# hellojialee/OffsetGuided

Measured on AMD Instinct MI355X. Metric: images/sec end-to-end (backbone+decode) @640x640 bs8; decoder-only ms/img, higher is better.
Workload: dtype f16

## Files before the change

include/og_decoder.h:

```cpp
#ifndef OG_DECODER_H
#define OG_DECODER_H

#include <stddef.h>
#include <stdint.h>

#ifdef __cplusplus
extern "C" {
#endif

#define OG_ABI_VERSION 4

#define OG_OK 0
#define OG_EINVAL (-1)
#define OG_ENOSPC (-2)
#define OG_EHIP (-3)
#define OG_EUNSUPPORTED (-4)

int og_abi_version(void);
const char *og_last_error(void);

int og_device_count(void);

int og_upsample_bicubic4_f32(const float *src, long planes, int h, int w, float *dst, void *stream);

// ... 82 lines not shown
int og_upsample2_add_bf16(void *up, const void *low, long n, int H, int W, int channels, void *stream);

int og_nchw_f32_to_nhwc_bf16(const float *src, void *dst, long N, int C, int H, int W, void *stream);
int og_nhwc_bf16_to_nchw_f32(const void *src, int src_channels, int first_channel, int channels, const float *bias,
                             float *dst, long N, int H, int W, void *stream);

int og_center_pad_normalize_u8(const unsigned char *img, int h, int w, int target_h, int target_w, const float *mean3,
                               const float *std3, const float *fill3, float *out, int *ltrb, void *stream);

int og_resize_cubic_u8(const unsigned char *src, int h, int w, unsigned char *dst, int new_h, int new_w, void *stream);

int og_shrink_mask_miss_u8(const unsigned char *mask, int N, int h, int w, int stride, unsigned char *out, void *stream);

int og_rescale_pad_normalize_u8(const unsigned char *img, int h, int w, int new_h, int new_w, int target_h, int target_w,
                                int corner_pad, const float *mean3, const float *std3, const float *fill3, float *out,
                                int *ltrb, void *stream);

int og_rescale_pad_normalize_batch_u8(const unsigned char *raw, const long *offsets, const int *hw4, int n, int target_h,
                                      int target_w, int corner_pad, const float *mean3, const float *std3, const float *fill3,
                                      float *out, int *ltrb, void *stream);

int og_stem7x7_bf16(const float *images, const void *w_packed, const float *bias, void *out, int N, int H, int W, int relu,
                    void *stream);

int og_conv3x3_bf16(const void *x, const void *w, const float *bias, const void *skip, void *out, int N, int H, int W,
                    int Cin, int Cout, int relu, void *workspace, size_t workspace_bytes, void *stream);
size_t og_conv3x3_workspace_bytes(long pixels, int Cin, int Cout);
size_t og_conv3x3_workspace_bytes_nhw(int N, int H, int W, int Cin, int Cout);
int og_conv2d_bf16(const void *x, const void *w, const float *bias, const void *skip, void *out, int N, int Hin, int Win,
                   int Cin, int Cout, int ksize, int stride, int relu, void *workspace, size_t workspace_bytes,
                   void *stream);
size_t og_conv2d_workspace_bytes(int N, int Hin, int Win, int Cin, int Cout, int ksize, int stride);
int og_conv2d_proj_bf16(const void *x, const void *w_cat, const float *bias, const void *x2, void *out, int N, int Hin,
                        int Win, int Cin, int Cout, int ksize, int stride, int H2, int W2, int Cin2, int stride2, int relu,
                        void *workspace, size_t workspace_bytes, void *stream);
size_t og_conv2d_proj_workspace_bytes(int N, int Hin, int Win, int Cin, int Cout, int ksize, int stride, int Cin2);
int og_conv_band_supported(int N, int Hin, int Win, int Cin, int Cout, int stride, int H2, int W2, int Cin2, int stride2);
int og_conv_band_pack_w16(const void *w, const void *w2, int Cin, int Cout, int Cin2, void *packed, void *stream);
int og_conv_band_bf16(const void *x, const void *w_packed, const float *bias, const void *skip, const void *x2, void *out, int N,
                      int Hin, int Win, int Cin, int Cout, int stride, int relu, int H2, int W2, int Cin2, int stride2, void *stream);
int og_conv_band_f16(const void *x, const void *w_packed, const float *bias, const void *skip, const void *x2, void *out, int N,
                     int Hin, int Win, int Cin, int Cout, int stride, int relu, int H2, int W2, int Cin2, int stride2, void *stream);
void og_conv_next_weights_hint(const void *w_next, size_t bytes);
int og_conv3x3_tiled_supported(int N, int H, int W, int Cin, int Cout);
int og_conv3x3_pack_w16(const void *w, int Cin, int Cout, int order, void *packed, void *stream);
size_t og_conv3x3_tiled_workspace_bytes(int N, int H, int W, int Cin, int Cout);
int og_conv3x3_tiled_bf16(const void *x, const void *w_packed, const float *bias, const void *skip, void *out, int N, int H,
                          int W, int Cin, int Cout, int relu, void *workspace, size_t workspace_bytes, void *stream);
int og_conv3x3_tiled_up2_bf16(const void *x, const void *w_packed, const float *bias, const void *skip, void *up, int N, int H,
                              int W, int Cin, int Cout, int relu, void *workspace, size_t workspace_bytes, void *stream);
int og_conv3x3s2_tiled_supported(int N, int Hin, int Win, int Cin, int Cout);
int og_conv3x3s2_tiled_bf16(const void *x, const void *w_packed, const float *bias, const void *skip, void *out, int N, int Hin,
                            int Win, int Cin, int Cout, int relu, void *stream);
int og_conv1x1_tiled_bf16(const void *x1, int C1, int H1, int W1, int stride1, const void *x2, int C2, int H2, int W2, int stride2,
                          const void *w_packed, const float *bias, const void *skip, void *out, int N, int H, int W, int Cout,
                          int relu, void *stream);
int og_conv1x1_heads_bf16(const void *x, int C, const void *w_packed, const float *bias, int N, int H, int W, int Cout, int n_heads,
                          const int *head_channels, float *const *outs, void *stream);
int og_bias_act_f16(void *x, const float *bias, const void *skip, long pixels, int channels, int relu, void *stream);
int og_upsample2_add_f16(void *up, const void *low, long n, int H, int W, int channels, void *stream);
int og_nchw_f32_to_nhwc_f16(const float *src, void *dst, long N, int C, int H, int W, void *stream);
int og_nhwc_f16_to_nchw_f32(const void *src, int src_channels, int first_channel, int channels, const float *bias,
                            float *dst, long N, int H, int W, void *stream);
int og_stem7x7_f16(const float *images, const void *w_packed, const float *bias, void *out, int N, int H, int W, int relu,
                   void *stream);
int og_conv3x3_f16(const void *x, const void *w, const float *bias, const void *skip, void *out, int N, int H, int W,
                   int Cin, int Cout, int relu, void *workspace, size_t workspace_bytes, void *stream);
int og_conv3x3_tiled_f16(const void *x, const void *w_packed, const float *bias, const void *skip, void *out, int N, int H,
                         int W, int Cin, int Cout, int relu, void *workspace, size_t workspace_bytes, void *stream);
int og_conv3x3_tiled_up2_f16(const void *x, const void *w_packed, const float *bias, const void *skip, void *up, int N, int H,
                         int W, int Cin, int Cout, int relu, void *workspace, size_t workspace_bytes, void *stream);
int og_conv3x3s2_tiled_f16(const void *x, const void *w_packed, const float *bias, const void *skip, void *out, int N, int Hin,
                           int Win, int Cin, int Cout, int relu, void *stream);
int og_conv1x1_tiled_f16(const void *x1, int C1, int H1, int W1, int stride1, const void *x2, int C2, int H2, int W2, int stride2,
                         const void *w_packed, const float *bias, const void *skip, void *out, int N, int H, int W, int Cout,
                         int relu, void *stream);
int og_conv1x1_heads_f16(const void *x, int C, const void *w_packed, const float *bias, int N, int H, int W, int Cout, int n_heads,
                         const int *head_channels, float *const *outs, void *stream);
int og_conv2d_f16(const void *x, const void *w, const float *bias, const void *skip, void *out, int N, int Hin, int Win,
                  int Cin, int Cout, int ksize, int stride, int relu, void *workspace, size_t workspace_bytes, void *stream);
int og_conv2d_proj_f16(const void *x, const void *w_cat, const float *bias, const void *x2, void *out, int N, int Hin,
                       int Win, int Cin, int Cout, int ksize, int stride, int H2, int W2, int Cin2, int stride2, int relu,
                       void *workspace, size_t workspace_bytes, void *stream);

int og_focal_l2_loss_f32(const float *pred, const float *gt, const unsigned char *mask_miss, int N, int C, long hw,
                         float tau, float gamma, float *sum, float *grad, void *stream);
int og_offset_l1_loss_f32(const float *pred, const float *gt, const float *gt_ps, const unsigned char *mask_miss, int N,
                          int C, long hw, float margin, int sqrt_re, float *sum_count, float *grad, void *stream);
int og_l2_loss_f32(const float *pred, const float *gt, const unsigned char *mask_miss, int N, int C, long hw, float *sum,
                   float *grad, void *stream);
int og_masked_l1_loss_f32(const float *pred, const float *gt, const unsigned char *mask_miss, int N, int C, long hw,
                          float margin, int sqrt_re, float *sum_count, float *grad, void *stream);
int og_vector_l1_loss_f32(const float *pred, const float *gt, const unsigned char *mask_miss, int N, int C, long hw,
                          float margin, int sqrt_re, float *sum_count, float *grad, void *stream);
int og_laplace_loss_f32(const float *pred, const float *gt, const float *logb, const unsigned char *mask_miss, int N, int C,
                        long hw, float margin, int sqrt_re, float *sum_count, float *grad, float *grad_logb, void *stream);

int og_encode_heatmaps_f32(const float *joints, const int32_t *n_persons, int N, int P, int n_kp, int in_w, int in_h,
                           int stride, int sigma, float clip_thre, float *hm, float *bg, void *stream);
int og_encode_jitter_f32(const float *joints, const int32_t *n_persons, int N, int P, int n_kp, int in_w, int in_h,
                         int stride, int fill_size, float *jit, void *stream);
int og_encode_offsets_f32(const float *joints, const int32_t *n_persons, int N, int P, int n_kp, const int32_t *jf,
                          const int32_t *jt, int L, int in_w, int in_h, int stride, int fill_size, float min_jscale,
                          const float *sigmas, float *off, float *scale, float *pscale, void *stream);

int og_draw_poses_u8(void *images, const float *poses, const int *n_persons, const int *skeleton,
// ... 93 lines not shown
```

offsetguided_amd/_lib.py:

```python
import ctypes as C
import os

import torch

_HERE = os.path.dirname(os.path.abspath(__file__))
LIB_PATH = os.path.join(_HERE, "libog_decoder.so")
if os.environ.get("OG_DECODER_LIB"):
    LIB_PATH = os.environ["OG_DECODER_LIB"]

OG_OK, OG_EINVAL, OG_ENOSPC, OG_EHIP, OG_EUNSUPPORTED = 0, -1, -2, -3, -4
ABI_VERSION = 4

_vp, _i, _l, _f, _d, _sz = C.c_void_p, C.c_int, C.c_long, C.c_float, C.c_double, C.c_size_t


class LimbsDesc(C.Structure):
    _fields_ = [("size", C.c_uint32), ("hmps", _vp), ("hm_lowres", _i), ("kp_perm", _vp), ("offs", _vp), ("off_lowres", _i), ("vector_nd", _i),
                ("limb_perm", _vp), ("reserve_mask", _vp), ("score_ksize", _i), ("scales", _vp), ("scales_mode", _i), ("jitter", _vp),
                ("jitter_mode", _i), ("N", _i), ("C", _i), ("H", _i), ("W", _i), ("jf", _vp), ("jt", _vp), ("L", _i), ("k", _i),
                ("thre_hmp", _f), ("min_len", _f), ("resize_factor", _f), ("topk_scores", _vp), ("topk_inds", _vp), ("limbs", _vp)]

    def __init__(self, **fields):
        super().__init__(size=C.sizeof(LimbsDesc), **{k: v.data_ptr() if isinstance(v, torch.Tensor) else v for k, v in fields.items()})

# ... 5 lines not shown

    def __init__(self, **fields):
        super().__init__(size=C.sizeof(CocoMaskDesc), **{k: v.data_ptr() if isinstance(v, torch.Tensor) else v for k, v in fields.items()})


SIGNATURES = {
    "og_abi_version": (_i, []),
    "og_last_error": (C.c_char_p, []),
    "og_device_count": (_i, []),
    "og_upsample_bicubic4_f32": (_i, [_vp, _l, _i, _i, _vp, _vp]),
    "og_upsample_bilinear4_f32": (_i, [_vp, _l, _i, _i, _vp, _vp]),
    "og_upsample_bicubic4_flip_f32": (_i, [_vp, _vp, _i, _i, _i, _i, _vp, _vp]),
    "og_hmp_nms_f32": (_i, [_vp, _l, _i, _i, _vp, _vp]),
    "og_hmp_nms_k_f32": (_i, [_vp, _l, _i, _i, _i, _vp, _vp]),
    "og_topk_channel_f32": (_i, [_vp, _l, _i, _i, _i, _vp, _vp, _vp, _sz, _vp]),
    "og_nms_topk_f32": (_i, [_vp, _l, _i, _i, _i, _vp, _vp, _vp, _sz, _vp]),
    "og_scored_offset_f32": (_i, [_vp, _vp, _i, _i, _i, _i, _i, _vp, _i, _vp, _vp]),
    "og_upsample_nms_topk_f32": (_i, [_vp, _l, _i, _i, _i, _vp, _vp, _vp, _sz, _vp]),
    "og_topk_workspace_bytes": (_sz, [_l, _i, _i, _i]),
    "og_collect_limbs_f32": (_i, [_vp, _vp, C.POINTER(LimbsDesc), _vp]),
    "og_generate_limbs_f32": (_i, [C.POINTER(LimbsDesc), _vp, _sz, _vp]),
    "og_generate_limbs_workspace_bytes": (_sz, [_i, _i, _i, _i, _i]),
    "og_greedy_group_f32": (_i, [_vp, _i, _i, _i, _vp, _vp, _i, _d, _f, _i, _i, _i, _vp, _vp, _vp, _vp, _sz, _vp]),
    "og_group_workspace_bytes": (_sz, [_i, _i, _i, _i, _i]),
    "og_flip_merge_f32": (_i, [_vp, _vp, _i, _i, _i, _i, _i, _vp, _vp, _vp, _vp, _vp, _vp]),
    "og_flip_cat_f32": (_i, [_vp, _vp, _i, _i, _i, _i, _i, _vp, _vp, _vp, _vp, _vp, _vp]),
    "og_flip_merge_heads_f32": (_i, [_vp, _vp, _i, _i, _i, _i, _vp, _vp, _vp, _vp]),
    "og_scale_accumulate_f32": (_i, [_vp, _vp, _i, _i, _i, _i, _i, _i, _vp, _vp, _vp, _vp, _i, _i, _i, _f, _vp, _vp, _vp]),
    "og_scale_accumulate_heads_f32": (_i, [_vp, _vp, _vp, _vp, _i, _i, _i, _i, _i, _i, _vp, _vp, _vp, _vp, _i, _i, _i, _f, _vp, _vp, _vp, _vp,
                                           _vp]),
    "og_bias_act_bf16": (_i, [_vp, _vp, _vp, _l, _i, _i, _vp]),
    "og_upsample2_add_bf16": (_i, [_vp, _vp, _l, _i, _i, _i, _vp]),
    "og_nchw_f32_to_nhwc_bf16": (_i, [_vp, _vp, _l, _i, _i, _i, _vp]),
    "og_nhwc_bf16_to_nchw_f32": (_i, [_vp, _i, _i, _i, _vp, _vp, _l, _i, _i, _vp]),
    "og_center_pad_normalize_u8": (_i, [_vp, _i, _i, _i, _i, _vp, _vp, _vp, _vp, _vp, _vp]),
    "og_resize_cubic_u8": (_i, [_vp, _i, _i, _vp, _i, _i, _vp]),
    "og_shrink_mask_miss_u8": (_i, [_vp, _i, _i, _i, _i, _vp, _vp]),
    "og_rescale_pad_normalize_u8": (_i, [_vp, _i, _i, _i, _i, _i, _i, _i, _vp, _vp, _vp, _vp, _vp, _vp]),
    "og_rescale_pad_normalize_batch_u8": (_i, [_vp, _vp, _vp, _i, _i, _i, _i, _vp, _vp, _vp, _vp, _vp, _vp]),
    "og_stem7x7_bf16": (_i, [_vp, _vp, _vp, _vp, _i, _i, _i, _i, _vp]),
    "og_conv3x3_bf16": (_i, [_vp, _vp, _vp, _vp, _vp, _i, _i, _i, _i, _i, _i, _vp, _sz, _vp]),
    "og_conv3x3_workspace_bytes": (_sz, [_l, _i, _i]),
    "og_conv3x3_workspace_bytes_nhw": (_sz, [_i, _i, _i, _i, _i]),
    "og_conv2d_bf16": (_i, [_vp, _vp, _vp, _vp, _vp, _i, _i, _i, _i, _i, _i, _i, _i, _vp, _sz, _vp]),
    "og_conv2d_workspace_bytes": (_sz, [_i, _i, _i, _i, _i, _i, _i]),
    "og_conv2d_proj_bf16": (_i, [_vp, _vp, _vp, _vp, _vp, _i, _i, _i, _i, _i, _i, _i, _i, _i, _i, _i, _i, _vp, _sz, _vp]),
    "og_conv2d_proj_workspace_bytes": (_sz, [_i, _i, _i, _i, _i, _i, _i, _i]),
    "og_conv_band_supported": (_i, [_i, _i, _i, _i, _i, _i, _i, _i, _i, _i]),
    "og_conv_band_pack_w16": (_i, [_vp, _vp, _i, _i, _i, _vp, _vp]),
    "og_conv_band_bf16": (_i, [_vp, _vp, _vp, _vp, _vp, _vp, _i, _i, _i, _i, _i, _i, _i, _i, _i, _i, _i, _vp]),
    "og_conv3x3_tiled_supported": (_i, [_i, _i, _i, _i, _i]),
    "og_conv3x3_pack_w16": (_i, [_vp, _i, _i, _i, _vp, _vp]),
    "og_conv3x3s2_tiled_supported": (_i, [_i, _i, _i, _i, _i]),
    "og_conv1x1_tiled_bf16": (_i, [_vp, _i, _i, _i, _i, _vp, _i, _i, _i, _i, _vp, _vp, _vp, _vp, _i, _i, _i, _i, _i, _vp]),
    "og_conv1x1_heads_bf16": (_i, [_vp, _i, _vp, _vp, _i, _i, _i, _i, _i, _vp, _vp, _vp]),
    "og_conv3x3s2_tiled_bf16": (_i, [_vp, _vp, _vp, _vp, _vp, _i, _i, _i, _i, _i, _i, _vp]),
    "og_conv3x3_tiled_workspace_bytes": (_sz, [_i, _i, _i, _i, _i]),
    "og_conv_next_weights_hint": (None, [_vp, _sz]),
    "og_conv3x3_tiled_bf16": (_i, [_vp, _vp, _vp, _vp, _vp, _i, _i, _i, _i, _i, _i, _vp, _sz, _vp]),
    "og_conv3x3_tiled_up2_bf16": (_i, [_vp, _vp, _vp, _vp, _vp, _i, _i, _i, _i, _i, _i, _vp, _sz, _vp]),
    "og_encode_heatmaps_f32": (_i, [_vp, _vp, _i, _i, _i, _i, _i, _i, _i, _f, _vp, _vp, _vp]),
    "og_encode_jitter_f32": (_i, [_vp, _vp, _i, _i, _i, _i, _i, _i, _i, _vp, _vp]),
    "og_encode_offsets_f32": (_i, [_vp, _vp, _i, _i, _i, _vp, _vp, _i, _i, _i, _i, _i, _f, _vp, _vp, _vp, _vp, _vp]),
    "og_focal_l2_loss_f32": (_i, [_vp, _vp, _vp, _i, _i, _l, _f, _f, _vp, _vp, _vp]),
    "og_offset_l1_loss_f32": (_i, [_vp, _vp, _vp, _vp, _i, _i, _l, _f, _i, _vp, _vp, _vp]),
    "og_l2_loss_f32": (_i, [_vp, _vp, _vp, _i, _i, _l, _vp, _vp, _vp]),
    "og_masked_l1_loss_f32": (_i, [_vp, _vp, _vp, _i, _i, _l, _f, _i, _vp, _vp, _vp]),
    "og_vector_l1_loss_f32": (_i, [_vp, _vp, _vp, _i, _i, _l, _f, _i, _vp, _vp, _vp]),
    "og_laplace_loss_f32": (_i, [_vp, _vp, _vp, _vp, _i, _i, _l, _f, _i, _vp, _vp, _vp, _vp]),
    "og_draw_poses_u8": (_i, [_vp, _vp, _vp, _vp, _vp, _i, _i, _i, _i, _i, _i, _i, _f, _f, _f, _vp]),
    "og_draw_heatmap_u8": (_i, [_vp, _vp, _vp, _i, _i, _i, _i, _i, _i, _f, _f, _f, _i, _vp]),
    "og_draw_segments_u8": (_i, [_vp, _vp, _vp, _i, _i, _i, _i, C.c_uint, C.c_uint, _f, _f, _f, _f, _vp]),
    "og_limbs_to_segments_f32": (_i, [_vp, _i, _i, _i, _i, _f, _vp, _vp, _vp]),
    "og_offsets_segments_capacity": (_l, [_i, _i, _i]),
    "og_offsets_to_segments_f32": (_i, [_vp, _vp, _i, _i, _i, _i, _i, _i, _i, _i, _f, _vp, _vp, _vp]),
    "og_warp_affine_batch_u8": (_i, [_vp, _vp, _vp, _i, _vp, _i, _vp, _vp, _vp, _vp, _vp, _vp]),
    "og_warp_affine_mask_u8": (_i, [_vp, _vp, _vp, _i, _vp, _i, _i, _vp, _vp]),
    "og_affine_joints_f32": (_i, [_vp, _vp, _i, _i, _i, _vp, _vp, _vp, _f, _f, _vp, _vp, _i, _vp, _vp]),
    "og_warp_affine_photo_batch_u8": (_i, [_vp, _vp, _vp, _i, _vp, _i, _vp, _vp, _vp, _vp, _vp, _vp, _vp]),
    "og_jpeg_roundtrip_batch_u8": (_i, [_vp, _i, _i, _vp, _i, _i, _vp, _vp, _vp, _vp, _vp]),
    "og_affine_joints_jitter_f32": (_i, [_vp, _vp, _i, _i, _i, _vp, _vp, _vp, _f, _f, _vp, _vp, _i, _vp, _vp, _vp, _vp, _vp, _vp]),
    "og_oks_matrix_f64": (_i, [_vp, _vp, _vp, _vp, _vp, _vp, _vp, _vp, _i, _i, _i, C.c_int64, _vp, _vp]),
    "og_oks_match_workspace_bytes": (_sz, [_i, _i, _i]),
    "og_oks_match_i32": (_i, [_vp, _vp, _vp, _vp, _vp, _vp, _vp, _vp, _vp, _i, _vp, _i, _i, _i, _i, C.c_int64, _vp, _vp, _vp, _vp, _sz, _vp]),
    "og_coco_mask_workspace_bytes": (_sz, [C.POINTER(CocoMaskDesc)]),
    "og_coco_masks_u8": (_i, [C.POINTER(CocoMaskDesc), _vp, _sz, _vp]),
    "og_optim_chunk_elems": (_i, []),
    "og_optim_workspace_bytes": (_sz, [_i]),
    "og_grad_sumsq_f32": (_i, [_vp, _vp, _i, _i, _vp, _sz, _vp]),
    "og_step_scale_f32": (_i, [_i, _vp, _f, _f, _vp, _sz, _vp]),
    "og_step_scale_amp_f32": (_i, [_i, _vp, _f, _f, _vp, _i, _f, _i, _f, _f, _vp, _sz, _vp]),
    "og_adam_step_f32": (_i, [_vp, _vp, _i, _i, _i, _vp, _f, _f, _f, _f, _f, _f, _f, _f, _f, _i, _vp]),
    "og_sgd_step_f32": (_i, [_vp, _vp, _i, _i, _i, _vp, _f, _f, _f, _i, _vp]),
}

for _name in [n for n in SIGNATURES if n.endswith('_bf16')]:
    SIGNATURES[_name[:-5] + '_f16'] = SIGNATURES[_name]
SIGNATURES['og_nhwc_f16_to_nchw_f32'] = SIGNATURES['og_nhwc_bf16_to_nchw_f32']

_lib = None


def lp(lib, stem, dtype):
    return getattr(lib, stem + ('_f16' if dtype == torch.float16 else '_bf16'))


# ... 188 lines not shown
```

offsetguided_amd/csrc/conv3x3.hip:

```cpp
#include <stdio.h>

#include <type_traits>

#include "lp_dtype.h"
#include "og_common.h"

namespace {

typedef lp8 bf16x8;
typedef float f32x4 __attribute__((ext_vector_type(4)));
typedef unsigned short u16x4 __attribute__((ext_vector_type(4)));
typedef unsigned short u16x8 __attribute__((ext_vector_type(8)));

constexpr int kZeroPageBytes = 256;

struct ConvArgs {
    const unsigned short *x;
    const unsigned short *w;
    const float *bias;
    const unsigned short *skip;
    unsigned short *out;
    unsigned short *up;
    float *partial;
    int *counters;
// ... 635 lines not shown
    return OG_OK;
}
}

OG_API int OG_LP_NAME(og_conv3x3_tiled)(const void *x, const void *w_packed, const float *bias, const void *skip, void *out, int N,
                                        int H, int W, int Cin, int Cout, int relu, void *workspace, size_t workspace_bytes,
                                        void *stream)
{
    return conv3x3_tiled_impl(OG_LP_STR("og_conv3x3_tiled"), x, w_packed, bias, skip, out, nullptr, N, H, W, Cin, Cout, relu, workspace,
                              workspace_bytes, stream);
}

OG_API int OG_LP_NAME(og_conv3x3_tiled_up2)(const void *x, const void *w_packed, const float *bias, const void *skip, void *up, int N,
                                            int H, int W, int Cin, int Cout, int relu, void *workspace, size_t workspace_bytes,
                                            void *stream)
{
    const char *name = OG_LP_STR("og_conv3x3_tiled_up2");
    OG_REQUIRE(up, OG_EINVAL, "%s: null pointer", name);
    OG_REQUIRE((long)N * H * W * 4 * Cout < (1l << 30), OG_EUNSUPPORTED, "%s: tensor too large (>= 2 GiB)", name);
    return conv3x3_tiled_impl(name, x, w_packed, bias, skip, nullptr, up, N, H, W, Cin, Cout, relu, workspace, workspace_bytes, stream);
}

OG_API int OG_LP_NAME(og_conv3x3s2_tiled)(const void *x, const void *w_packed, const float *bias, const void *skip, void *out,
                                          int N, int Hin, int Win, int Cin, int Cout, int relu, void *stream)
{
    const char *name = OG_LP_STR("og_conv3x3s2_tiled");
    OG_REQUIRE(x && w_packed && bias && out, OG_EINVAL, "%s: null pointer", name);
    ConvArgs h = {};
    const int rc = tiled_fill(name, h, x, w_packed, bias, skip, out, N, Hin, Win, 2, Cin, Cout, relu);
    if (rc != OG_OK) return rc;
    const int kind = og_conv3x3s2_tiled_supported(N, Hin, Win, Cin, Cout);
    OG_REQUIRE(kind != 0, OG_EUNSUPPORTED,
               "%s: needs Cout %% 128 == 0, Cin %% 64 == 0 and an output of 8k x 16k pixels or 2k x 40 (got %dx%d -> %dx%d, %d -> %d)", name,
               Hin, Win, h.H, h.W, Cin, Cout);
    h.warm = og_take_warm_hint();
#define S2_LAUNCH(TW_, TH_, WM_)                                                                                      \
    do {                                                                                                              \
        static OgAttrOnce attr_;                                                                                      \
        if (attr_.need())                                                                                             \
            (void)hipFuncSetAttribute((const void *)conv3x3s2_tiled_kernel<TW_, TH_, WM_>,                            \
                                      hipFuncAttributeMaxDynamicSharedMemorySize, kS2LdsBytes);                       \
        const long blocks_ = (long)N * (h.H / TH_) * (h.W / TW_) * h.n_tiles;                                         \
        hipLaunchKernelGGL((conv3x3s2_tiled_kernel<TW_, TH_, WM_>), dim3((unsigned)blocks_), dim3(256), kS2LdsBytes,  \
                           (hipStream_t)stream, h);                                                                   \
    } while (0)
    if (kind == 2) S2_LAUNCH(40, 2, 1);
    else S2_LAUNCH(16, 8, 2);
#undef S2_LAUNCH
    OG_LAUNCH_CHECK(name);
    return OG_OK;
}

static int pw_fill(const char *name, PwArgs &a, const void *x1, int C1, int H1, int W1, int s1, const void *x2, int C2, int H2, int W2,
                   int s2, const void *w_packed, const float *bias, int N, int H, int W, int Cout, int bn)
{
    OG_REQUIRE(x1 && w_packed, OG_EINVAL, "%s: null pointer", name);
    OG_REQUIRE(N > 0 && H > 0 && W > 0 && (s1 == 1 || s1 == 2) && (!x2 || s2 == 1 || s2 == 2), OG_EINVAL, "%s: bad shape", name);
    OG_REQUIRE(C1 > 0 && C1 % 64 == 0 && (!x2 || (C2 > 0 && C2 % 64 == 0)) && Cout % bn == 0, OG_EUNSUPPORTED,
               "%s: input channels must be multiples of 64 and Cout of %d (got %d + %d -> %d)", name, bn, C1, x2 ? C2 : 0, Cout);
    OG_REQUIRE((H - 1) * s1 < H1 && (W - 1) * s1 < W1, OG_EINVAL, "%s: the strided output reaches outside the input", name);
    OG_REQUIRE(!x2 || (C2 == C1 && H2 == H1 && W2 == W1 && s2 == s1), OG_EUNSUPPORTED,
               "%s: a second input must have the shape and stride of the first", name);
    const long M = (long)N * H * W;
    OG_REQUIRE((long)N * H1 * W1 * C1 < (1l << 30) && (!x2 || (long)N * H2 * W2 * C2 < (1l << 30)) && M * Cout < (1l << 30), OG_EUNSUPPORTED,
               "%s: tensor too large (>= 2 GiB)", name);
    a.x1 = (const unsigned short *)x1; a.x2 = (const unsigned short *)x2; a.w = (const unsigned short *)w_packed; a.bias = bias;
    a.N = N; a.H = H; a.W = W; a.Cout = Cout; a.M = (int)M;
    a.C1 = C1; a.H1 = H1; a.W1 = W1; a.s1 = s1;
    a.C2 = x2 ? C2 : 0; a.H2 = H2; a.W2 = W2; a.s2 = s2;
    a.x1_bytes = (int)((long)N * H1 * W1 * C1 * 2);
    a.x2_bytes = x2 ? (int)((long)N * H2 * W2 * C2 * 2) : 0;
    a.w_bytes = Cout * (a.C1 + a.C2) * 2;
    a.n_tiles = Cout / bn;
    a.items = (int)((M + 255) / 256) * a.n_tiles;
#ifdef OG_PW_STAMPS
    a.stamps = g_stamps;
#endif
    return OG_OK;
}

static long pw_blocks(const PwArgs &a)
{
    constexpr int kPerCu = 2;
    const long unit = 8l * a.n_tiles;
    const long cap = (long)kPerCu * og_cu_count() / unit * unit;
    if (cap <= 0 || a.items <= cap || a.items % 8 != 0) return a.items;
    return cap;
}

template <int BN, int MODE>
static void pw_launch(const PwArgs &a, long blocks, int lds_bytes, void *stream)
{
    static OgAttrOnce attr_;
    if (lds_bytes > 64 * 1024 && attr_.need()) {
        (void)hipFuncSetAttribute((const void *)conv1x1_tiled_kernel<BN, MODE, 2>, hipFuncAttributeMaxDynamicSharedMemorySize, lds_bytes);
        (void)hipFuncSetAttribute((const void *)conv1x1_tiled_kernel<BN, MODE, 1>, hipFuncAttributeMaxDynamicSharedMemorySize, lds_bytes);
    }
    if (((a.C1 + a.C2) >> 6) % 2 == 0)
        hipLaunchKernelGGL((conv1x1_tiled_kernel<BN, MODE, 2>), dim3((unsigned)blocks), dim3(256), lds_bytes, (hipStream_t)stream, a);
    else
        hipLaunchKernelGGL((conv1x1_tiled_kernel<BN, MODE, 1>), dim3((unsigned)blocks), dim3(256), lds_bytes, (hipStream_t)stream, a);
}

OG_API int OG_LP_NAME(og_conv1x1_tiled)(const void *x1, int C1, int H1, int W1, int stride1, const void *x2, int C2, int H2, int W2,
                                        int stride2, const void *w_packed, const float *bias, const void *skip, void *out, int N,
                                        int H, int W, int Cout, int relu, void *stream)
{
    const char *name = OG_LP_STR("og_conv1x1_tiled");
    OG_REQUIRE(out, OG_EINVAL, "%s: null pointer", name);
    PwArgs a = {};
    const int rc = pw_fill(name, a, x1, C1, H1, W1, stride1, x2, C2, H2, W2, stride2, w_packed, bias, N, H, W, Cout, 128);
    if (rc != OG_OK) return rc;
    a.skip = (const unsigned short *)skip; a.out = (unsigned short *)out; a.relu = relu;
    constexpr int lds_ = 256 * (2 * 128 + 16);
    static_assert(lds_ >= 3 * 2 * 128 * 64 && 2 * lds_ <= 160 * 1024, "LDS");
    pw_launch<128, 0>(a, pw_blocks(a), lds_, stream);
    OG_LAUNCH_CHECK(name);
    return OG_OK;
}

OG_API int OG_LP_NAME(og_conv1x1_heads)(const void *x, int C, const void *w_packed, const float *bias, int N, int H, int W, int Cout,
                                        int n_heads, const int *head_channels, float *const *outs, void *stream)
{
    const char *name = OG_LP_STR("og_conv1x1_heads");
    OG_REQUIRE(head_channels && outs && bias, OG_EINVAL, "%s: null pointer", name);
    OG_REQUIRE(n_heads >= 1 && n_heads <= 4, OG_EUNSUPPORTED, "%s: 1 to 4 heads", name);
    PwArgs a = {};
    const int rc = pw_fill(name, a, x, C, H, W, 1, nullptr, 0, 0, 0, 1, w_packed, bias, N, H, W, Cout, 64);
    if (rc != OG_OK) return rc;
    int c = 0;
    for (int i = 0; i < 4; ++i) {
        a.first[i] = c;
        if (i < n_heads) {
            OG_REQUIRE(head_channels[i] > 0 && outs[i], OG_EINVAL, "%s: bad head %d", name, i);
            c += head_channels[i];
            a.outf[i] = outs[i];
        }
    }
    a.first[4] = c;
    for (int i = n_heads; i < 4; ++i) a.first[i] = c;
    OG_REQUIRE(c <= Cout, OG_EINVAL, "%s: the heads have %d channels, the packed weight %d", name, c, Cout);
    constexpr int lds_ = 3 * 2 * 64 * 64;
    pw_launch<64, 1>(a, a.items, lds_, stream);
    OG_LAUNCH_CHECK(name);
    return OG_OK;
}
```

offsetguided_amd/csrc/conv3x3_tiled.inc:

```

template <int N, int I = 0, class F>
__device__ __forceinline__ void og_static_for(F &&f)
{
    if constexpr (I < N) {
        f(std::integral_constant<int, I>());
        og_static_for<N, I + 1>(f);
    }
}

__host__ __device__ __forceinline__ constexpr int tiled_swz(int row) { return (4 - ((row >> 2) & 3)) & 3; }

__global__ void __launch_bounds__(256)
conv3x3_pack_kernel(const unsigned short *w, unsigned short *packed, int Cin, int Cout, int order)
{
    const long slot = (long)blockIdx.x * 256 + threadIdx.x;
    const int taps = order >= 2 ? 1 : 9, rows = order == 3 ? 64 : 128;
    const long total = (long)Cout * taps * Cin / 8;
    if (slot >= total) return;
    const int chunks = Cin >> 5;
    const int in_stage = (int)(slot % (rows * 4));
    long stage = slot / (rows * 4);
    const int kS2[9] = {0, 2, 6, 8, 3, 5, 1, 7, 4};
    const int tslot = (int)(stage % taps), tap = order == 1 ? kS2[tslot] : tslot;
    stage /= taps;
// ... 641 lines not shown
    int q = 0;
#pragma unroll 1
    for (; q + 2 < chunks; q += 2) {
        chunk_body(yes, even, q);
        chunk_body(yes, odd, q + 1);
    }
    chunk_body(yes, even, q);
    chunk_body(no, odd, q + 1);

    constexpr int kOPitch = BN * 2 + 16, kTilePx = TW * TH, kPerPx = BN / 8;
    static_assert(kTilePx * kOPitch <= kRing * kBBytes + 3 * kABytes, "output staging must fit the LDS of the main loop");
    f32x4 bias_r[NT];
#pragma unroll
    for (int n = 0; n < NT; ++n) bias_r[n] = *reinterpret_cast<const f32x4 *>(a.bias + n0 + (wn * NT + n) * 16 + fk * 4);
    __syncthreads();
#pragma unroll
    for (int m = 0; m < MT; ++m) {
        const int px = (wm * MT + m) * 16 + fcol;
#pragma unroll
        for (int n = 0; n < NT; ++n) {
            const int cl = (wn * NT + n) * 16 + fk * 4;
            const f32x4 v = acc[n][m] + bias_r[n];
            u16x4 o;
#pragma unroll
            for (int jj = 0; jj < 4; ++jj) o[jj] = f2bf(a.relu ? fmaxf(v[jj], 0.f) : v[jj]);
            *reinterpret_cast<u16x4 *>(lds + px * kOPitch + cl * 2) = o;
        }
    }
    __syncthreads();
    const size_t tile_px = (size_t)(img * a.H + y0) * a.W + x0;
    for (int g = tid; g < kTilePx * kPerPx; g += 256) {
        const int px = g / kPerPx, cg = g % kPerPx;
        const size_t off = (tile_px + (size_t)(px / TW) * a.W + (px % TW)) * a.Cout + n0 + cg * 8;
        *reinterpret_cast<u16x8 *>(a.out + off) = *reinterpret_cast<const u16x8 *>(lds + px * kOPitch + cg * 16);
    }
    og_warm_sink(warm_v);
}

struct PwArgs {
    const unsigned short *x1, *x2;
    const unsigned short *w;
    const float *bias;
    const unsigned short *skip;
    unsigned short *out;
    float *outf[4];
    int first[5];
    int N, H, W, Cout, M;
    int C1, H1, W1, s1, C2, H2, W2, s2;
    int x1_bytes, x2_bytes, w_bytes, n_tiles, relu;
    int items;
    unsigned long long *stamps;
};

template <int BN, int MODE, int D = 1>
__global__ void __launch_bounds__(256, 2)
conv1x1_tiled_kernel(PwArgs a)
{
    constexpr int MT = 4, NT = BN / 16, kHalf = BN * 64, kStage = 2 * kHalf, kRing = 3;
    constexpr int PW = kStage / 4096;
    static_assert(PW >= 1 && kRing * kStage <= 64 * 1024, "LDS");
    extern __shared__ __attribute__((aligned(1024))) unsigned char lds[];

    const int tid = threadIdx.x, wave = tid >> 6, lane = tid & 63;
#ifdef OG_PW_STAMPS
#define PW_STAMP(i)                                                                                            \
    do {                                                                                                       \
        unsigned long long t_;                                                                                 \
        asm volatile("s_memrealtime %0\n\ts_waitcnt lgkmcnt(0)" : "=s"(t_));                                   \
        if (a.stamps) a.stamps[((size_t)stamp_id * 4 + wave) * 8 + (i)] = t_;                                   \
    } while (0)
#else
#define PW_STAMP(i)
#endif
    int stamp_id = blockIdx.x;
    (void)stamp_id;
    const int fcol = lane & 15, fk = lane >> 4;
    for (int vid = blockIdx.x; vid < a.items; vid += gridDim.x) {
    const int item = (a.items & 7) == 0 && (gridDim.x & 7) == 0 ? og_xcd_remap(vid, a.items) : vid;
    const int nt_i = item % a.n_tiles, m0 = (item / a.n_tiles) * 256, n0 = nt_i * BN;
    if (vid != (int)blockIdx.x) __syncthreads();
    stamp_id = vid;
    PW_STAMP(0);
    const int steps1 = a.C1 >> 6, steps = steps1 + (a.C2 >> 6);

    typedef int rsrc_t __attribute__((ext_vector_type(4)));
    auto mk_rsrc = [](const void *p, int bytes) {
        const uint64_t b = reinterpret_cast<uint64_t>(p);
        rsrc_t r;
        r[0] = (int)(uint32_t)b;
        r[1] = (int)((uint32_t)(b >> 32) & 0xffffu);
        r[2] = bytes;
        r[3] = 0x00020000;
        return r;
    };
    const rsrc_t x1r = mk_rsrc(a.x1, a.x1_bytes), x2r = mk_rsrc(a.x2 ? a.x2 : a.x1, a.x2 ? a.x2_bytes : 0);
    const __amdgpu_buffer_rsrc_t wr = __builtin_amdgcn_make_buffer_rsrc(const_cast<unsigned short *>(a.w), 0, a.w_bytes, 0x00020000);
    uint32_t p1[MT];
    if (a.s1 == 1 && a.H1 == a.H && a.W1 == a.W) {
#pragma unroll
        for (int m = 0; m < MT; ++m) {
            const int p = m0 + wave * 64 + m * 16 + fcol;
            p1[m] = p < a.M ? (uint32_t)p * (uint32_t)(a.C1 * 2) + (uint32_t)(fk * 16) : kOobOffset;
        }
    } else {
#pragma unroll
        for (int m = 0; m < MT; ++m) {
            const int p = m0 + wave * 64 + m * 16 + fcol;
            const int t = p / a.W, x = p - t * a.W, n = t / a.H, y = t - n * a.H;
            p1[m] = p < a.M ? (uint32_t)((((n * a.H1 + y * a.s1) * a.W1 + x * a.s1) * a.C1) * 2 + fk * 16) : kOobOffset;
        }
    }
    typedef unsigned int u32x4 __attribute__((ext_vector_type(4)));
    auto load_px = [&](int s, auto half_tag, bf16x8 (&pf)[MT]) {
        constexpr int HALF = decltype(half_tag)::value;
        const bool second = s >= steps1;
        const uint32_t soff = (uint32_t)((second ? s - steps1 : s) * 128);
        const uint32_t beyond = s >= steps ? kOobOffset : 0u;
        const rsrc_t r = second ? x2r : x1r;
        og_static_for<MT>([&](auto m_tag) {
            constexpr int m = decltype(m_tag)::value;
            u32x4 v;
            asm volatile("buffer_load_dwordx4 %0, %1, %2, %3 offen offset:%4" : "=v"(v) : "v"(p1[m] | beyond), "s"(r), "s"(soff), "i"(HALF * 64));
            pf[m] = __builtin_bit_cast(bf16x8, v);
        });
    };
    const int piece = wave * 64 * 16;
// ... 72 lines not shown
        bias_r[n] = a.bias ? *reinterpret_cast<const f32x4 *>(a.bias + n0 + n * 16 + fk * 4) : (f32x4){0.f, 0.f, 0.f, 0.f};
    if constexpr (MODE == 0) {
        constexpr int kOPitch = BN * 2 + 16, kPerPx = BN / 8;
        __syncthreads();
#pragma unroll
        for (int m = 0; m < MT; ++m) {
            __builtin_amdgcn_sched_barrier(0);
            const int px = wave * 64 + m * 16 + fcol, p = m0 + px;
#pragma unroll
            for (int n = 0; n < NT; ++n) {
                f32x4 v = acc[n][m] + bias_r[n];
                if (a.skip && p < a.M) {
                    const u16x4 sk = *reinterpret_cast<const u16x4 *>(a.skip + (size_t)p * a.Cout + n0 + n * 16 + fk * 4);
#pragma unroll
                    for (int j = 0; j < 4; ++j) v[j] += bf2f(sk[j]);
                }
                u16x4 o;
#pragma unroll
                for (int j = 0; j < 4; ++j) o[j] = f2bf(a.relu ? fmaxf(v[j], 0.f) : v[j]);
                *reinterpret_cast<u16x4 *>(lds + px * kOPitch + (n * 16 + fk * 4) * 2) = o;
            }
        }
        __syncthreads();
#pragma unroll 4
        for (int g = tid; g < 256 * kPerPx; g += 256) {
            const int px = g / kPerPx, cg = g % kPerPx, p = m0 + px;
            if (p < a.M)
                *reinterpret_cast<u16x8 *>(a.out + (size_t)p * a.Cout + n0 + cg * 8) = *reinterpret_cast<const u16x8 *>(lds + px * kOPitch + cg * 16);
        }
    } else {
#pragma unroll
        for (int m = 0; m < MT; ++m) {
            __builtin_amdgcn_sched_barrier(0);
            const int p = m0 + wave * 64 + m * 16 + fcol;
            if (p >= a.M) continue;
            const int hw = a.H * a.W, img = p / hw, pix = p - img * hw;
#pragma unroll
            for (int n = 0; n < NT; ++n) {
                const int co = n0 + n * 16 + fk * 4;
                const f32x4 v = acc[n][m] + bias_r[n];
#pragma unroll
                for (int j = 0; j < 4; ++j) {
                    const int c = co + j;
#pragma unroll
                    for (int hd = 0; hd < 4; ++hd)
                        if (c >= a.first[hd] && c < a.first[hd + 1])
                            a.outf[hd][((size_t)img * (a.first[hd + 1] - a.first[hd]) + (c - a.first[hd])) * hw + pix] = v[j];
                }
            }
        }
    }
    PW_STAMP(5);
    }
#undef PW_STAMP
}
```

Measured before the change: 1411.

## Add 1x1 conv kernel with full-Cout tile to read activations once

```diff
diff --git a/include/og_decoder.h b/include/og_decoder.h
--- a/include/og_decoder.h
+++ b/include/og_decoder.h
@@ -158,6 +158,7 @@
 int og_conv3x3s2_tiled_supported(int N, int Hin, int Win, int Cin, int Cout);
 int og_conv3x3s2_tiled_bf16(const void *x, const void *w_packed, const float *bias, const void *skip, void *out, int N, int Hin,
                             int Win, int Cin, int Cout, int relu, void *stream);
+int og_conv1x1_tiled_plan(int N, int H, int W, int Cout, int two_inputs, int *plan);
 int og_conv1x1_tiled_bf16(const void *x1, int C1, int H1, int W1, int stride1, const void *x2, int C2, int H2, int W2, int stride2,
                           const void *w_packed, const float *bias, const void *skip, void *out, int N, int H, int W, int Cout,
                           int relu, void *stream);
diff --git a/offsetguided_amd/_lib.py b/offsetguided_amd/_lib.py
--- a/offsetguided_amd/_lib.py
+++ b/offsetguided_amd/_lib.py
@@ -81,6 +81,7 @@
     "og_conv3x3_tiled_supported": (_i, [_i, _i, _i, _i, _i]),
     "og_conv3x3_pack_w16": (_i, [_vp, _i, _i, _i, _vp, _vp]),
     "og_conv3x3s2_tiled_supported": (_i, [_i, _i, _i, _i, _i]),
+    "og_conv1x1_tiled_plan": (_i, [_i, _i, _i, _i, _i, C.POINTER(_i)]),
     "og_conv1x1_tiled_bf16": (_i, [_vp, _i, _i, _i, _i, _vp, _i, _i, _i, _i, _vp, _vp, _vp, _vp, _i, _i, _i, _i, _i, _vp]),
     "og_conv1x1_heads_bf16": (_i, [_vp, _i, _vp, _vp, _i, _i, _i, _i, _i, _vp, _vp, _vp]),
     "og_conv3x3s2_tiled_bf16": (_i, [_vp, _vp, _vp, _vp, _vp, _i, _i, _i, _i, _i, _i, _vp]),
diff --git a/offsetguided_amd/csrc/conv3x3.hip b/offsetguided_amd/csrc/conv3x3.hip
--- a/offsetguided_amd/csrc/conv3x3.hip
+++ b/offsetguided_amd/csrc/conv3x3.hip
@@ -711,7 +711,7 @@
 }
 
 static int pw_fill(const char *name, PwArgs &a, const void *x1, int C1, int H1, int W1, int s1, const void *x2, int C2, int H2, int W2,
-                   int s2, const void *w_packed, const float *bias, int N, int H, int W, int Cout, int bn)
+                   int s2, const void *w_packed, const float *bias, int N, int H, int W, int Cout, int bn, int item_px = 256)
 {
     OG_REQUIRE(x1 && w_packed, OG_EINVAL, "%s: null pointer", name);
     OG_REQUIRE(N > 0 && H > 0 && W > 0 && (s1 == 1 || s1 == 2) && (!x2 || s2 == 1 || s2 == 2), OG_EINVAL, "%s: bad shape", name);
@@ -731,7 +731,7 @@
     a.x2_bytes = x2 ? (int)((long)N * H2 * W2 * C2 * 2) : 0;
     a.w_bytes = Cout * (a.C1 + a.C2) * 2;
     a.n_tiles = Cout / bn;
-    a.items = (int)((M + 255) / 256) * a.n_tiles;
+    a.items = (int)((M + item_px - 1) / item_px) * a.n_tiles;
 #ifdef OG_PW_STAMPS
     a.stamps = g_stamps;
 #endif
@@ -761,19 +761,56 @@
         hipLaunchKernelGGL((conv1x1_tiled_kernel<BN, MODE, 1>), dim3((unsigned)blocks), dim3(256), lds_bytes, (hipStream_t)stream, a);
 }
 
+struct PwShape { int px, bn, lds; };
+static PwShape pw_shape(int Cout, bool two_inputs)
+{
+    constexpr int lds_ = 256 * (2 * 128 + 16);
+    static_assert(lds_ >= 3 * 2 * 128 * 64 && 2 * lds_ <= 160 * 1024 && 2 * pw_once_lds_bytes() <= 160 * 1024, "LDS");
+#ifndef OG_PW_ONCE
+#define OG_PW_ONCE 1
+#endif
+    if (Cout == kPwOnceBn && (OG_PW_ONCE == 2 || (OG_PW_ONCE == 1 && two_inputs))) return {kPwOncePx, kPwOnceBn, pw_once_lds_bytes()};
+    return {256, 128, lds_};
+}
+
+#ifndef OG_DT_F16
+OG_API int og_conv1x1_tiled_plan(int N, int H, int W, int Cout, int two_inputs, int *plan)
+{
+    if (!plan || N <= 0 || H <= 0 || W <= 0 || Cout <= 0 || Cout % 128 || (long)N * H * W * Cout >= (1l << 30)) return OG_EUNSUPPORTED;
+    const PwShape sh = pw_shape(Cout, two_inputs != 0);
+    PwArgs a = {};
+    a.n_tiles = Cout / sh.bn;
+    a.items = (int)(((long)N * H * W + sh.px - 1) / sh.px) * a.n_tiles;
+    plan[0] = sh.px; plan[1] = sh.bn; plan[2] = a.items; plan[3] = (int)pw_blocks(a); plan[4] = sh.lds;
+    return OG_OK;
+}
+#endif
+
 OG_API int OG_LP_NAME(og_conv1x1_tiled)(const void *x1, int C1, int H1, int W1, int stride1, const void *x2, int C2, int H2, int W2,
                                         int stride2, const void *w_packed, const float *bias, const void *skip, void *out, int N,
                                         int H, int W, int Cout, int relu, void *stream)
 {
     const char *name = OG_LP_STR("og_conv1x1_tiled");
     OG_REQUIRE(out, OG_EINVAL, "%s: null pointer", name);
+    const PwShape sh = pw_shape(Cout, x2 != nullptr);
     PwArgs a = {};
-    const int rc = pw_fill(name, a, x1, C1, H1, W1, stride1, x2, C2, H2, W2, stride2, w_packed, bias, N, H, W, Cout, 128);
+    const int rc = pw_fill(name, a, x1, C1, H1, W1, stride1, x2, C2, H2, W2, stride2, w_packed, bias, N, H, W, Cout, sh.bn, sh.px);
     if (rc != OG_OK) return rc;
     a.skip = (const unsigned short *)skip; a.out = (unsigned short *)out; a.relu = relu;
-    constexpr int lds_ = 256 * (2 * 128 + 16);
-    static_assert(lds_ >= 3 * 2 * 128 * 64 && 2 * lds_ <= 160 * 1024, "LDS");
-    pw_launch<128, 0>(a, pw_blocks(a), lds_, stream);
+    if (sh.bn == kPwOnceBn) {
+        static OgAttrOnce attr_;
+        if (attr_.need()) {
+            (void)hipFuncSetAttribute((const void *)conv1x1_once_kernel<2>, hipFuncAttributeMaxDynamicSharedMemorySize, sh.lds);
+            (void)hipFuncSetAttribute((const void *)conv1x1_once_kernel<1>, hipFuncAttributeMaxDynamicSharedMemorySize, sh.lds);
+        }
+        const long blocks = pw_blocks(a);
+        if (((a.C1 + a.C2) >> 6) % 2 == 0)
+            hipLaunchKernelGGL(conv1x1_once_kernel<2>, dim3((unsigned)blocks), dim3(256), sh.lds, (hipStream_t)stream, a);
+        else
+            hipLaunchKernelGGL(conv1x1_once_kernel<1>, dim3((unsigned)blocks), dim3(256), sh.lds, (hipStream_t)stream, a);
+    } else {
+        pw_launch<128, 0>(a, pw_blocks(a), sh.lds, stream);
+    }
     OG_LAUNCH_CHECK(name);
     return OG_OK;
 }
diff --git a/offsetguided_amd/csrc/conv3x3_tiled.inc b/offsetguided_amd/csrc/conv3x3_tiled.inc
--- a/offsetguided_amd/csrc/conv3x3_tiled.inc
+++ b/offsetguided_amd/csrc/conv3x3_tiled.inc
@@ -717,16 +717,6 @@
     unsigned long long *stamps;
 };
 
-template <int BN, int MODE, int D = 1>
-__global__ void __launch_bounds__(256, 2)
-conv1x1_tiled_kernel(PwArgs a)
-{
-    constexpr int MT = 4, NT = BN / 16, kHalf = BN * 64, kStage = 2 * kHalf, kRing = 3;
-    constexpr int PW = kStage / 4096;
-    static_assert(PW >= 1 && kRing * kStage <= 64 * 1024, "LDS");
-    extern __shared__ __attribute__((aligned(1024))) unsigned char lds[];
-
-    const int tid = threadIdx.x, wave = tid >> 6, lane = tid & 63;
 #ifdef OG_PW_STAMPS
 #define PW_STAMP(i)                                                                                            \
     do {                                                                                                       \
@@ -737,6 +727,17 @@
 #else
 #define PW_STAMP(i)
 #endif
+
+template <int BN, int MODE, int D = 1>
+__global__ void __launch_bounds__(256, 2)
+conv1x1_tiled_kernel(PwArgs a)
+{
+    constexpr int MT = 4, NT = BN / 16, kHalf = BN * 64, kStage = 2 * kHalf, kRing = 3;
+    constexpr int PW = kStage / 4096;
+    static_assert(PW >= 1 && kRing * kStage <= 64 * 1024, "LDS");
+    extern __shared__ __attribute__((aligned(1024))) unsigned char lds[];
+
+    const int tid = threadIdx.x, wave = tid >> 6, lane = tid & 63;
     int stamp_id = blockIdx.x;
     (void)stamp_id;
     const int fcol = lane & 15, fk = lane >> 4;
@@ -915,5 +916,164 @@
     }
     PW_STAMP(5);
     }
+}
+
+constexpr int kPwOncePx = 128, kPwOnceBn = 256;
+constexpr int pw_once_lds_bytes()
+{
+    constexpr int ring = 5 * kPwOnceBn * 64, staging = kPwOncePx * (kPwOnceBn * 2 + 16);
+    return ring > staging ? ring : staging;
+}
+
+template <int D>
+__global__ void __launch_bounds__(256, 2)
+conv1x1_once_kernel(PwArgs a)
+{
+    constexpr int BN = kPwOnceBn, MT = 2, NT = BN / 16, kImg = 128 * 64, kStage = 2 * kImg, DH = 2 * D, kRing = DH + 1;
+    constexpr int PW = kStage / 4096;
+    static_assert(kRing * kStage <= pw_once_lds_bytes() && 2 * pw_once_lds_bytes() <= 160 * 1024, "LDS: two workgroups per CU");
+    extern __shared__ __attribute__((aligned(1024))) unsigned char lds[];
+
+    const int tid = threadIdx.x, wave = tid >> 6, lane = tid & 63;
+    int stamp_id = blockIdx.x;
+    (void)stamp_id;
+    const int fcol = lane & 15, fk = lane >> 4;
+    for (int vid = blockIdx.x; vid < a.items; vid += gridDim.x) {
+    const int item = (a.items & 7) == 0 && (gridDim.x & 7) == 0 ? og_xcd_remap(vid, a.items) : vid;
+    const int nt_i = item % a.n_tiles, m0 = (item / a.n_tiles) * kPwOncePx, n0 = nt_i * BN;
+    if (vid != (int)blockIdx.x) __syncthreads();
+    stamp_id = vid;
+    PW_STAMP(0);
+    const int steps1 = a.C1 >> 6, steps = steps1 + (a.C2 >> 6), halves = 2 * steps;
+
+    typedef int rsrc_t __attribute__((ext_vector_type(4)));
+    auto mk_rsrc = [](const void *p, int bytes) {
+        const uint64_t b = reinterpret_cast<uint64_t>(p);
+        rsrc_t r;
+        r[0] = (int)(uint32_t)b;
+        r[1] = (int)((uint32_t)(b >> 32) & 0xffffu);
+        r[2] = bytes;
+        r[3] = 0x00020000;
+        return r;
+    };
+    const rsrc_t x1r = mk_rsrc(a.x1, a.x1_bytes), x2r = mk_rsrc(a.x2 ? a.x2 : a.x1, a.x2 ? a.x2_bytes : 0);
+    const __amdgpu_buffer_rsrc_t wr = __builtin_amdgcn_make_buffer_rsrc(const_cast<unsigned short *>(a.w), 0, a.w_bytes, 0x00020000);
+    uint32_t p1[MT];
+    if (a.s1 == 1 && a.H1 == a.H && a.W1 == a.W) {
+#pragma unroll
+        for (int m = 0; m < MT; ++m) {
+            const int p = m0 + wave * 32 + m * 16 + fcol;
+            p1[m] = p < a.M ? (uint32_t)p * (uint32_t)(a.C1 * 2) + (uint32_t)(fk * 16) : kOobOffset;
+        }
+    } else {
+#pragma unroll
+        for (int m = 0; m < MT; ++m) {
+            const int p = m0 + wave * 32 + m * 16 + fcol;
+            const int t = p / a.W, x = p - t * a.W, n = t / a.H, y = t - n * a.H;
+            p1[m] = p < a.M ? (uint32_t)((((n * a.H1 + y * a.s1) * a.W1 + x * a.s1) * a.C1) * 2 + fk * 16) : kOobOffset;
+        }
+    }
+    typedef unsigned int u32x4 __attribute__((ext_vector_type(4)));
+    auto load_px = [&](int h, auto half_tag, bf16x8 (&pf)[MT]) {
+        constexpr int HALF = decltype(half_tag)::value;
+        const int s = h >> 1;
+        const bool second = s >= steps1;
+        const uint32_t soff = (uint32_t)((second ? s - steps1 : s) * 128);
+        const uint32_t beyond = h >= halves ? kOobOffset : 0u;
+        const rsrc_t r = second ? x2r : x1r;
+        og_static_for<MT>([&](auto m_tag) {
+            constexpr int m = decltype(m_tag)::value;
+            u32x4 v;
+            asm volatile("buffer_load_dwordx4 %0, %1, %2, %3 offen offset:%4" : "=v"(v) : "v"(p1[m] | beyond), "s"(r), "s"(soff), "i"(HALF * 64));
+            pf[m] = __builtin_bit_cast(bf16x8, v);
+        });
+    };
+    const int piece = wave * 64 * 16;
+    const uint32_t w_voff = (uint32_t)tid * 16;
+    const uint32_t w_tile_bytes = (uint32_t)(halves * kImg);
+    const uint32_t w_tile = (uint32_t)(2 * nt_i) * w_tile_bytes;
+    auto issue_b = [&](int h, int ring) {
+        const uint32_t voff = w_voff | (h >= halves ? kOobOffset : 0u);
+#pragma unroll
+        for (int i = 0; i < PW; ++i)
+            blds16(wr, voff, w_tile + (uint32_t)(i >> 1) * w_tile_bytes + h * kImg + (i & 1) * 4096, lds + ring * kStage + piece + i * 4096);
+    };
+    const int w_rd = fcol * 64 + ((fk ^ tiled_swz(fcol)) << 4);
+
+    f32x4 acc[NT][MT];
+#pragma unroll
+    for (int n = 0; n < NT; ++n)
+#pragma unroll
+        for (int m = 0; m < MT; ++m) acc[n][m] = (f32x4){0.f, 0.f, 0.f, 0.f};
+    bf16x8 pf[DH][MT], wf[4];
+    og_static_for<DH>([&](auto i_tag) {
+        constexpr int i = decltype(i_tag)::value;
+        issue_b(i, i);
+        load_px(i, std::integral_constant<int, i & 1>(), pf[i]);
+    });
+    PW_STAMP(1);
+    auto half_body = [&](auto set_tag, int h) {
+        constexpr int SET = decltype(set_tag)::value;
+        wait_vm_lgkm0<(DH - 1) * (PW + MT)>();
+        if (h == 0) PW_STAMP(2);
+        __builtin_amdgcn_s_barrier();
+        __builtin_amdgcn_sched_barrier(0);
+        issue_b(h + DH, (h + DH) % kRing);
+        const unsigned char *wB = lds + (h % kRing) * kStage;
+#pragma unroll
+        for (int nb = 0; nb < NT; nb += 4) {
+#pragma unroll
+            for (int n = 0; n < 4; ++n) wf[n] = *reinterpret_cast<const bf16x8 *>(wB + w_rd + (nb + n) * 1024);
+#pragma unroll
+            for (int n = 0; n < 4; ++n)
+#pragma unroll
+                for (int m = 0; m < MT; ++m) acc[nb + n][m] = OG_LP_MFMA(wf[n], pf[SET][m], acc[nb + n][m]);
+        }
+        __builtin_amdgcn_sched_barrier(0);
+        load_px(h + DH, std::integral_constant<int, SET & 1>(), pf[SET]);
+    };
+#pragma unroll 1
+    for (int h = 0; h < halves; h += DH)
+        og_static_for<DH>([&](auto i_tag) { half_body(i_tag, h + decltype(i_tag)::value); });
+    PW_STAMP(3);
+    wait_vm_lgkm0<0>();
+    PW_STAMP(4);
+
+    constexpr int kOPitch = BN * 2 + 16, kPerPx = BN / 8;
+    __syncthreads();
+#pragma unroll
+    for (int nh = 0; nh < NT; nh += 8) {
+        f32x4 bias_r[8];
+#pragma unroll
+        for (int n = 0; n < 8; ++n)
+            bias_r[n] = a.bias ? *reinterpret_cast<const f32x4 *>(a.bias + n0 + (nh + n) * 16 + fk * 4) : (f32x4){0.f, 0.f, 0.f, 0.f};
+#pragma unroll
+        for (int m = 0; m < MT; ++m) {
+            __builtin_amdgcn_sched_barrier(0);
+            const int px = wave * 32 + m * 16 + fcol, p = m0 + px;
+#pragma unroll
+            for (int n = 0; n < 8; ++n) {
+                f32x4 v = acc[nh + n][m] + bias_r[n];
+                if (a.skip && p < a.M) {
+                    const u16x4 sk = *reinterpret_cast<const u16x4 *>(a.skip + (size_t)p * a.Cout + n0 + (nh + n) * 16 + fk * 4);
+#pragma unroll
+                    for (int j = 0; j < 4; ++j) v[j] += bf2f(sk[j]);
+                }
+                u16x4 o;
+#pragma unroll
+                for (int j = 0; j < 4; ++j) o[j] = f2bf(a.relu ? fmaxf(v[j], 0.f) : v[j]);
+                *reinterpret_cast<u16x4 *>(lds + px * kOPitch + ((nh + n) * 16 + fk * 4) * 2) = o;
+            }
+        }
+    }
+    __syncthreads();
+#pragma unroll 4
+    for (int g = tid; g < kPwOncePx * kPerPx; g += 256) {
+        const int px = g / kPerPx, cg = g % kPerPx, p = m0 + px;
+        if (p < a.M)
+            *reinterpret_cast<u16x8 *>(a.out + (size_t)p * a.Cout + n0 + cg * 8) = *reinterpret_cast<const u16x8 *>(lds + px * kOPitch + cg * 16);
+    }
+    PW_STAMP(5);
+    }
+}
 #undef PW_STAMP
-}
```

Result: no change. 1416 (median of 6 runs) (+0.4%).
